# andrewmilson/ecfft

Hardware: AMD Instinct MI355X
Metric: secp256k1 Fp field-mul/s, ENTER+EXIT at n=2^20 (higher is better)
Workload: dtype u256; 1 GPU; secp256k1::Fp n=2^20 ENTER+EXIT (BASELINE.json configs[2]); n=1048576, field=secp256k1, parallelism=1 independent polynomial(s), one per GPU, no collective, inputs=device-resident (HBM) before the timed region, steps=449, warmup=5

## Files before the change

### ecfft_amd/csrc/device_tree.h

```cpp
#pragma once
#include <hip/hip_runtime.h>
#include <vector>
#include <set>
#include <map>
#include <mutex>
#include <atomic>
#include <cstdio>
#include <cstdlib>
#include <new>
#include <algorithm>
#include "kernels.h"
#include "host_curve.h"
#include "transport.h"

namespace ecfft {

#ifdef ECFFT_TEST_HOOKS
inline const char* ab_env(const char* name) { return getenv(name); }
#else
inline const char* ab_env(const char*) { return nullptr; }
#endif

#define ECFFT_HIP_TRY(x)                                                                   \
    do { hipError_t e_ = (x); if (e_ != hipSuccess) {                                      \
// ... 68 lines not shown
public:
    using E = typename F::elem;
    using TE = typename F::telem;
    using Tree = LevelTables<F>;

    ~DeviceChain() { release(); }

    size_t size() const { return N_; }
    unsigned log_size() const { return L_; }
    const Tree& tree(unsigned log_m) const { return trees_[log_m]; }
    const Tree& tree_at(unsigned log_m) const { return (ovr_tree_ && ovr_tree_->log_m == log_m) ? *ovr_tree_ : trees_[log_m]; }
    const HostTree<F>& host() const { return host_; }
    int exit_cores() const { return exit3_ ? 3 : 4; }
    int exit_low_cores() const { return exit3_ && kExitLowForm == 3 && !exit_low4_ ? 3 : 4; }
    int sym_bfly() const { return !sym_ ? 0 : (sym_general_kernels_ ? 2 : 1); }
    int low_map(int dir) const {
        if (trees_.size() > 5 && trees_[5].low32_A[dir]) return 32;
        if (trees_.size() > 4 && trees_[4].low16_A[dir]) return 16;
        return 0;
    }
    const E* f_device() const { return f_; }
    std::mutex& lock() { return mu_; }
#ifdef ECFFT_TEST_HOOKS
    static std::atomic<int>& test_fail_build_rank() { static std::atomic<int> r{-1}; return r; }
#endif
    Profiler& profiler() const { return prof_; }

    bool build(HostTree<F>&& ht, int device) {
        host_ = std::move(ht);
        N_ = host_.n; L_ = ilog2(N_); device_ = device;
// ... 522 lines not shown
    static constexpr unsigned kLogTileMax = (sizeof(E) == 32) ? ECFFT_LOG_TILE_BYTES - 5 : ECFFT_LOG_TILE_BYTES - 2;
#ifndef ECFFT_COL_STAGES
#define ECFFT_COL_STAGES 9
#endif
#ifndef ECFFT_LOG_COL_TILE_BYTES
#define ECFFT_LOG_COL_TILE_BYTES 15
#endif
#ifndef ECFFT_COL_MIN_LOGC
#define ECFFT_COL_MIN_LOGC 1
#endif
#ifndef ECFFT_COL_STAGES_4B
#define ECFFT_COL_STAGES_4B 9
#endif
    static constexpr unsigned kColStages = sizeof(E) == 4 ? ECFFT_COL_STAGES_4B : ECFFT_COL_STAGES;
    static constexpr bool kSymKernels = sizeof(E) == 32 && ECFFT_SYM_BFLY != 0;
    static constexpr unsigned kLogColTileMax = (sizeof(E) == 32) ? ECFFT_LOG_COL_TILE_BYTES - 5 : ECFFT_LOG_COL_TILE_BYTES - 2;
    struct NextLoad { int ld_mode; const TE* ld_tbl; double extra_first; };
    struct EnterFuse { const E* src; E* dst; double extra; };
    bool extend_core(unsigned log_m, IoDesc<F> io, E* buf, size_t total, int srcpar, hipStream_t s,
                     double extra_first = 0.0, double extra_last = 0.0, unsigned k_begin = 0,
                     const NextLoad* next_ld = nullptr, bool skip_first_col = false, const EnterFuse* ef = nullptr) const {
        const Tree& T = tree_at(log_m);
        size_t e = T.e; unsigned le = ilog2(e);
        int tgt = 1 - srcpar;
        const bool symk = kSymKernels && sym_kernels();
        unsigned tz = (unsigned)__builtin_ctzll((unsigned long long)total);
        unsigned log_tile = tz < kLogTileMax ? tz : kLogTileMax;
        const bool small = small_launch(total) && !ef_small_off_;
        if (small && log_tile > kLogLowSmall) log_tile = kLogLowSmall;
        unsigned k_first = le > log_tile ? le - log_tile : 0;
// ... 547 lines not shown
        enter_rec(in, X, n / 2, s, sA, depth - 1, next_side);
        double w = tblw_; tblw_ = 0.0; enter_rec(in + n / 2, X + n / 2, n / 2, s2, sB, depth - 1, next_side); tblw_ = w;
        (void)hipEventRecord(ev_join_[me], s2); (void)hipStreamWaitEvent(s, ev_join_[me], 0);
        enter_levels(X, out, n, 1, s, sA, ln, ln);
    }
    static size_t scratch_need(size_t n, unsigned depth) { return depth == 0 ? 3 * n : n + 2 * scratch_need(n / 2, depth - 1) > 4 * n ? n + 2 * scratch_need(n / 2, depth - 1) : 4 * n; }
    void enter_levels(const E* in, E* out, size_t n, size_t count, hipStream_t s, E* base, unsigned l_begin, unsigned l_end) const {
        const size_t nt = n * count;
        E* bufA = base; E* bufB = base + nt; E* work = base + 2 * nt;
        const E* src = in;
        unsigned l0 = l_begin;
        const unsigned ll = log_low_for(nt);
        if (l_begin == 1 && l_end >= ll) {
            E* dst = (l_end == ll && out != in) ? out : bufA;
            double bytes = 0; for (unsigned l = 1; l <= ll; ++l) bytes += enter_level_alg_bytes(nt, l);
            if (ll == kLogLow)
                ECFFT_LAUNCH(KC_FUSED_ENTER, bytes, (k_enter_low<F, (int)kLogLow>), dim3((unsigned)(nt >> kLogLow)), dim3(kBlockLds),
                             2 * (sizeof(E) << kLogLow), s, dst, src, (const Tree*)d_trees_);
            else
                ECFFT_LAUNCH(KC_FUSED_ENTER, bytes, (k_enter_low<F, (int)kLogLowSmall, 2 * (int)kBlockLowSmall>), dim3((unsigned)(nt >> kLogLowSmall)), dim3(2 * kBlockLowSmall),
                             2 * (sizeof(E) << kLogLowSmall), s, dst, src, (const Tree*)d_trees_);
            src = dst; l0 = ll + 1;
        }
        for (unsigned l = l0; l <= l_end; ++l) {
            const Tree& T = trees_[l];
            size_t e = T.e;
            E* dst = (l == l_end && out != in) ? out : (src == bufA ? bufB : bufA);
            IoDesc<F> io = io_plain(src, work); io.ld_mode = LD_SCALE; io.ld_tbl = T.winv[0];
            EnterFuse ef{src, dst, sizeof(E) * (3.0 * nt + 2.0 * e * tblw_)};
            extend_core(l, io, work, nt, 0, s, 0.0, 0.0, 0, nullptr, false, &ef);
            src = dst;
// ... 6 lines not shown
    }
    double exit_level_alg_bytes(size_t n, unsigned l) const {
        double e = (double)((size_t)1 << (l - 1));
        return sizeof(E) * (8.0 * (l - 1) * (double)n + 8.5 * (double)n + tblw_ * (32.0 * (e - 1) + 8.5 * e));
    }
#ifndef ECFFT_SPLIT_MIN_LOG
#define ECFFT_SPLIT_MIN_LOG 19
#endif
#ifndef ECFFT_EXIT_CORES
#define ECFFT_EXIT_CORES 3
#endif
#ifndef ECFFT_EXIT_LOW_CORES
#define ECFFT_EXIT_LOW_CORES 3
#endif
    static constexpr int kExitLowForm = (ECFFT_EXIT_CORES == 4 || ECFFT_EXIT_LOW_CORES == 4) ? 4 : 3;
    static constexpr unsigned kSplitMinLog = ECFFT_SPLIT_MIN_LOG;
#ifndef ECFFT_SPLIT_DEPTH
#define ECFFT_SPLIT_DEPTH 1
#endif
#ifndef ECFFT_NT_STORE_MAX_LOG
#define ECFFT_NT_STORE_MAX_LOG 0
#endif
    static constexpr unsigned kNtStoreMaxLog = ECFFT_NT_STORE_MAX_LOG;
    static constexpr unsigned kSplitDepth = ECFFT_SPLIT_DEPTH;
    static constexpr int kMaxSides = 7;
    static constexpr unsigned kLogLow = (sizeof(E) == 32) ? 10 : 13;
    static constexpr unsigned kLogLowSmall = 8, kBlockLowSmall = 128, kSmallTiles = 256;
    unsigned small_tiles_max() const {
        static const int v = ab_env("ECFFT_SMALL_TILES_MAX") ? atoi(ab_env("ECFFT_SMALL_TILES_MAX")) : -1;
        return v >= 0 ? (unsigned)v : (in_halves_ ? kSmallTiles : 2 * kSmallTiles);
// ... 67 lines not shown
            bool f2 = extend_core(l, io_plain(G, G), G, nh, 1, s, 0.0, 0.0, 0, &nl3, f1);
            IoDesc<F> io3 = io_plain(G, G);
            io3.ld_mode = LD_SCALE; io3.ld_tbl = T.C1;
            io3.st_mode = ST_AXPBY; io3.st_a = T.NB2; io3.st_b = T.D1; io3.aux = H; io3.aux_stride = 1; io3.aux_off = 0; io3.aux_out = nullptr;
            bool f3 = extend_core(l, io3, G, nh, 0, s, f2 ? 0.0 : se * (3.0 * n + 3.0 * ee), se * (1.5 * n + 2.0 * ee), 0, &nl4, f2);
            IoDesc<F> io4 = io_plain(G, dst);
            io4.st_mode = ST_EXIT_SPLIT; io4.st_a = T.w[0]; io4.st_b = T.xie; io4.aux = cur; io4.aux_stride = 2; io4.aux_off = 0;
            extend_core(l, io4, G, nh, 1, s, 0.0, se * (1.5 * n + 0.5 * ee), 0, nullptr, f3);
            cur = dst;
        }
        if (l_to == 1 && l_from >= ll) {
            E* dst = out != in ? out : (cur == bufA ? bufB : bufA);
            double bytes = 0; for (unsigned l = 1; l <= ll; ++l) bytes += exit_level_alg_bytes(n, l);
            const bool low3 = exit_low_cores() == 3;
            if (ll == kLogLow) {
                if (low3) ECFFT_LAUNCH(KC_FUSED_EXIT, bytes, (k_exit_low<F, (int)kLogLow, (int)kBlockLds, kExitLowForm>), dim3((unsigned)(n >> kLogLow)), dim3(kBlockLds),
                                       2 * (sizeof(E) << kLogLow), s, dst, cur, (const Tree*)d_trees_);
                else ECFFT_LAUNCH(KC_FUSED_EXIT, bytes, (k_exit_low<F, (int)kLogLow, (int)kBlockLds, 4>), dim3((unsigned)(n >> kLogLow)), dim3(kBlockLds),
                                  2 * (sizeof(E) << kLogLow), s, dst, cur, (const Tree*)d_trees_);
            } else {
                if (low3) ECFFT_LAUNCH(KC_FUSED_EXIT, bytes, (k_exit_low<F, (int)kLogLowSmall, (int)kBlockLowSmall, kExitLowForm>), dim3((unsigned)(n >> kLogLowSmall)), dim3(kBlockLowSmall),
                                       2 * (sizeof(E) << kLogLowSmall), s, dst, cur, (const Tree*)d_trees_);
                else ECFFT_LAUNCH(KC_FUSED_EXIT, bytes, (k_exit_low<F, (int)kLogLowSmall, (int)kBlockLowSmall, 4>), dim3((unsigned)(n >> kLogLowSmall)), dim3(kBlockLowSmall),
                                  2 * (sizeof(E) << kLogLowSmall), s, dst, cur, (const Tree*)d_trees_);
            }
            cur = dst;
        }
        if (cur != out) (void)hipMemcpyAsync(out, cur, n * sizeof(E), hipMemcpyDeviceToDevice, s);
    }

    bool poly_mul(const E* a, size_t na, const E* b, size_t nb, E* out, size_t count, hipStream_t s) {
// ... 2523 lines not shown
                         ~StripeScope() { ch->stripe_stage_ = nullptr; ch->stripe_bytes_ = 0; } };
    bool stripe_off_ = ab_env("ECFFT_NO_STRIPE") != nullptr;
    size_t stripe_gain_ = ab_env("ECFFT_STRIPE_MIN_GAIN") ? (size_t)atoll(ab_env("ECFFT_STRIPE_MIN_GAIN")) : ~(size_t)0;
    bool q2_split_ = ab_env("ECFFT_SPLIT_Q2_SPLIT") != nullptr;
    bool col256_off_ = ab_env("ECFFT_NO_COL256") != nullptr;
    bool row256_off_ = ab_env("ECFFT_NO_ROW256") != nullptr;
    bool ef_small_off_ = ab_env("ECFFT_NO_SMALL_TILES") != nullptr;
    bool exit4_ = ECFFT_EXIT_CORES == 4 || ab_env("ECFFT_EXIT_FOUR_CORES") != nullptr;
    bool exit3_ = false;
    bool exit_low4_ = ab_env("ECFFT_EXIT_LOW_FOUR_CORES") != nullptr;
    E* crit_ = nullptr;
    bool sym_ = false;
    bool sym_off_ = ab_env("ECFFT_NO_SYM_BFLY") != nullptr;
    bool sym_general_kernels_ = ab_env("ECFFT_SYM_BFLY_GENERAL_KERNELS") != nullptr;
    bool sym_kernels() const { return sym_ && !sym_general_kernels_; }
};

}
```

### ecfft_amd/csrc/ecfft_capi.hip

```cpp
#include <hip/hip_runtime.h>
#include <cstring>
#include <memory>
#include <new>
#include "device_tree.h"
#include "wire_parse.h"
#include "../../include/ecfft_hip.h"
#ifdef ECFFT_TEST_HOOKS
#include "../../include/ecfft_hip_hooks.h"
#endif

using namespace ecfft;

struct ecfft_ctx {
    int field;
    int device;
    std::unique_ptr<DeviceChain<Secp256k1>> secp;
    std::unique_ptr<DeviceChain<M31>> m31;
    void* stage = nullptr;
    size_t stage_bytes = 0;
    hipEvent_t last_op = nullptr;
    ~ecfft_ctx() { if (stage) (void)hipFree(stage); if (last_op) (void)hipEventDestroy(last_op); }
};

namespace {
// ... 1510 lines not shown
int ecfft_ctx_low_map(const ecfft_ctx* ctx, int dir) {
    if (!ctx || dir < 0 || dir > 1 || ctx->field != ECFFT_FIELD_SECP256K1 || !ctx->secp) return 0;
    return ctx->secp->low_map(dir);
}
int ecfft_ctx_exit_cores(const ecfft_ctx* ctx) {
    if (!ctx) return 0;
    return ctx->secp ? ctx->secp->exit_cores() : ctx->m31 ? ctx->m31->exit_cores() : 0;
}
int ecfft_ctx_exit_low_cores(const ecfft_ctx* ctx) {
    if (!ctx) return 0;
    return ctx->secp ? ctx->secp->exit_low_cores() : ctx->m31 ? ctx->m31->exit_low_cores() : 0;
}
int ecfft_ctx_sym_bfly(const ecfft_ctx* ctx) {
    if (!ctx) return -1;
    return ctx->secp ? ctx->secp->sym_bfly() : ctx->m31 ? ctx->m31->sym_bfly() : -1;
}

#endif
int ecfft_mul_ceiling(int field, int device, int waves_per_simd, double* mul_per_s) {
    return with_field(field, [&](auto tag) { return run_mul_ceiling<typename decltype(tag)::type>(device, waves_per_simd, mul_per_s); });
}

int ecfft_device_alloc(int device, size_t bytes, void** out) {
    if (!out) return ECFFT_ERR_BAD_ARG;
    *out = nullptr;
    if (!have_device(device)) return ECFFT_ERR_HIP;
    DeviceGuard dev(device);
    if (!dev.ok) return ECFFT_ERR_HIP;
    return hipMalloc(out, bytes ? bytes : 1) == hipSuccess ? ECFFT_OK : ECFFT_ERR_HIP;
}
// ... 447 lines not shown
```

### ecfft_amd/csrc/kernels.h

```cpp
#pragma once
#include <hip/hip_runtime.h>
#include <stdint.h>
#include <stddef.h>
#include <type_traits>
#include "mfma_blk16.h"
#include "curve_points.h"

namespace ecfft {

constexpr int kBlock = 256;

__device__ __forceinline__ void lds_barrier() { asm volatile("s_waitcnt lgkmcnt(0)\n\ts_barrier" ::: "memory"); }
#ifndef ECFFT_WAVE_LOCAL
#define ECFFT_WAVE_LOCAL 1
#endif
__device__ __forceinline__ void wave_local_sync() {
#if ECFFT_WAVE_LOCAL == 2
    asm volatile("s_waitcnt lgkmcnt(0)" ::: "memory");
#elif ECFFT_WAVE_LOCAL == 1
    __builtin_amdgcn_fence(__ATOMIC_ACQ_REL, "wavefront");
    asm volatile("" ::: "memory");
#else
    lds_barrier();
#endif
// ... 504 lines not shown
}

template <class F, int EPT, int BLK>
__device__ __forceinline__ void lds_extend_fast(typename F::elem* a, const typename F::telem* __restrict__ np0, const typename F::telem* __restrict__ dinv,
                                                const typename F::telem* __restrict__ p0, const typename F::telem* __restrict__ p1,
                                                const typename F::telem* __restrict__ inner, size_t e64, uint32_t log_span, uint32_t tid) {
    const uint32_t e = (uint32_t)e64;
    constexpr uint32_t LOG_EPT = EPT == 16 ? 4 : 3;
    const uint32_t upper = log_span > LOG_EPT ? log_span - LOG_EPT : 0;
    if (upper) flat_stages<F, true, EPT, BLK>(a, np0, dinv, e, LOG_EPT, upper, tid);
    tail_stages<F, EPT, BLK>(a, np0, dinv, p0, p1, inner, e, log_span, tid);
    if (upper) flat_stages<F, false, EPT, BLK>(a, p0, p1, e, LOG_EPT, upper, tid);
    __syncthreads();
}

template <class F, bool DEC, bool SYM = false>
__device__ __forceinline__ void row_stages_pipe(typename F::elem* tile, const typename F::telem* __restrict__ ta, const typename F::telem* __restrict__ tb,
                                                uint32_t e, int lh_from, int lh_to, uint32_t tid, int lh_after = 99) {
    using E = typename F::elem;
    using TE = typename F::telem;
    if (DEC ? lh_from < lh_to : lh_from > lh_to) return;
    auto geom = [&](int lh, uint32_t& idx, uint32_t& ti) {
        const uint32_t h = 1u << lh, i = tid & (h - 1);
        idx = ((tid >> lh) << (lh + 1)) + i; ti = e - 2 * h + i;
    };
    uint32_t idx, ti;
    geom(lh_from, idx, ti);
    if constexpr (SYM) {
        const TE* __restrict__ tk = DEC ? tb : ta;
        TE nk = ldt(tk, ti);
#pragma unroll 1
        for (int lh = lh_from; DEC ? lh >= lh_to : lh <= lh_to; lh += DEC ? -1 : 1) {
            const TE t = nk;
            const uint32_t lo = idx, up = idx + (1u << lh);
            E a = tile[lo], b = tile[up];
            sym_bfly<F, DEC>(a, b, t);
            tile[lo] = a; tile[up] = b;
            if (lh != lh_to) { geom(lh + (DEC ? -1 : 1), idx, ti); nk = ldt(tk, ti); }
            const int nxt = lh != lh_to ? lh + (DEC ? -1 : 1) : lh_after;
            if (wave_local_lh(lh) && wave_local_lh(nxt)) wave_local_sync(); else lds_barrier();
        }
        return;
    }
    TE na = ldt(ta, ti), nb = ldt(tb, ti);
#pragma unroll 1
    for (int lh = lh_from; DEC ? lh >= lh_to : lh <= lh_to; lh += DEC ? -1 : 1) {
        const TE t0 = na, t1 = nb;
        const uint32_t lo = idx, up = idx + (1u << lh);
        const E a = tile[lo], b = tile[up];
        if (DEC) { const E q1 = F::tmul(t1, F::sub(b, a)); tile[lo] = F::tmul_add(t0, q1, a); tile[up] = q1; }
        else { const E o0 = F::tmul_add(t0, b, a), o1 = F::tmul_add(t1, b, a); tile[lo] = o0; tile[up] = o1; }
        if (lh != lh_to) { geom(lh + (DEC ? -1 : 1), idx, ti); na = ldt(ta, ti); nb = ldt(tb, ti); }
        const int nxt = lh != lh_to ? lh + (DEC ? -1 : 1) : lh_after;
// ... 827 lines not shown
        const uint32_t lh = log_e - k - 1, h = 1u << lh;
        const bool hi = (tid >> lh) & 1u;
        const uint32_t off = (uint32_t)(e - 2 * (size_t)h) + (tid & (h - 1));
        TE t; if (act) t = hi ? ldt(p1, off) : ldt(p0, off);
        const E xp = partner(h);
        if (act) {
            const E A = lane_sel<F>(hi, xp, x), B = lane_sel<F>(hi, x, xp);
            x = F::tmul_add(t, B, A);
        }
    }
    __syncthreads();
    if (act) lds_put<F, SWZ>(a, tid, x);
    __syncthreads();
}

template <class F, int BLK = kBlockLds, bool SWZ = false>
__device__ __forceinline__ void lds_extend_core(typename F::elem* a, uint32_t len, uint32_t log_e, const LevelTables<F>& T, int srcpar) {
    using E = typename F::elem;
    uint32_t tid_ = threadIdx.x;
#if ECFFT_CORE_OPAQUE_TID
    if constexpr (sizeof(E) == 32) asm volatile("" : "+v"(tid_));
#endif
    const uint32_t tid = tid_, npairs = len >> 1;
    const size_t e = (size_t)1 << log_e;
    const int tgt = 1 - srcpar;
    const uint8_t* bA = nullptr; const unsigned long long* bK = nullptr;
    if constexpr (sizeof(E) == 32 && BLK == 512) {
        if (log_e >= 4 && (len == 512u || (len & 1023u) == 0)) { bA = T.blk16_A[srcpar]; bK = T.blk16_K[srcpar]; }
    }
    if constexpr (sizeof(E) == 32 && (BLK == 256 || BLK == 128)) {
        if (log_e >= 4 && len == (uint32_t)BLK) { bA = T.blk16_A[srcpar]; bK = T.blk16_K[srcpar]; }
    }
    if constexpr (sizeof(E) == 32 && ECFFT_REG_ENGINE) {
        if (len <= (uint32_t)BLK && (len & 63u) == 0) {
            reg_extend32<F, BLK, SWZ>(a, len, log_e, 0, T.c0t[srcpar], T.dinv[srcpar], T.p0[tgt], T.p1[tgt], T.inner[srcpar], tid, len == (uint32_t)BLK ? bA : nullptr, bK);
            return;
        }
    }
    if constexpr (SWZ) __builtin_trap();
    if constexpr (sizeof(E) == 32) {
        if (len == BLK) {
            const uint32_t g = tid & (npairs - 1);
            const bool hi = tid >= npairs;
            const uint32_t k_inner = log_e ? log_e - 1 : 0;
            for (uint32_t k = 0; k < k_inner; ++k) {
                const uint32_t lh = log_e - k - 1, h = 1u << lh, i = g & (h - 1), idx = ((g >> lh) << (lh + 1)) + i;
// ... 21 lines not shown
                a[idx + (hi ? h : 0)] = F::tmul_add(t, y, x);
                __syncthreads();
            }
            return;
        }
    }
    if constexpr (sizeof(E) == 4) {
        if (len == BLK * 16) { lds_extend_fast<F, 16, BLK>(a, T.np0[srcpar], T.dinv[srcpar], T.p0[tgt], T.p1[tgt], T.inner[srcpar], e, log_e, tid); return; }
        if (len == BLK * 8) { lds_extend_fast<F, 8, BLK>(a, T.np0[srcpar], T.dinv[srcpar], T.p0[tgt], T.p1[tgt], T.inner[srcpar], e, log_e, tid); return; }
    }
    const uint32_t k_inner = log_e ? log_e - 1 : 0;
    bool mfma = false;
    if constexpr (sizeof(E) == 32 && BLK == 512) mfma = bA != nullptr && (len & 1023u) == 0;
    const uint32_t k_dec_end = mfma ? log_e - 4 : k_inner;
    const bool wl = sizeof(E) == 32 && 2 * npairs > (uint32_t)BLK;
    for (uint32_t k = 0; k < k_dec_end; ++k) {
        const uint32_t lh = log_e - k - 1, h = 1u << lh;
        stage_sweep<F, true, BLK>(a, T.np0[srcpar] + (e - 2 * (size_t)h), T.dinv[srcpar] + (e - 2 * (size_t)h), lh, npairs, tid, T.c0t[srcpar] + (e - 2 * (size_t)h));
        if (wl && wave_local_lh((int)lh) && (k + 1 < k_dec_end || !mfma)) wave_local_sync(); else __syncthreads();
    }
    if constexpr (sizeof(E) == 32 && BLK == 512) {
        if (mfma) {
            Blk16::APre pre = Blk16::prefetch(bA, tid);
            __builtin_amdgcn_sched_barrier(0);
            Blk16::to_operand_form<BLK>(a, len, tid);
#pragma unroll 1
            for (uint32_t o = 0; o < len; o += Blk16::kSub) {
                if (o) { pre = Blk16::prefetch(bA, tid); __builtin_amdgcn_sched_barrier(0); }
                Blk16::phase(a + o, bA, bK, tid, pre);
            }
            Blk16::from_swizzled<BLK>(a, len, tid);
        }
    }
    if (log_e > 0 && !mfma) {
        const typename F::telem c0 = ldt(T.inner[srcpar], 0u), c1 = ldt(T.inner[srcpar], 1u);
        for (uint32_t g = tid; g < npairs; g += BLK) {
            E x = a[2 * g], y = a[2 * g + 1];
            E d = F::sub(y, x);
            a[2 * g] = F::tmul_add(c0, d, x);
            a[2 * g + 1] = F::tmul_add(c1, d, x);
        }
        if (wl && ECFFT_WAVE_LOCAL && k_dec_end > 0) wave_local_sync(); else __syncthreads();
    }
    for (uint32_t k = k_dec_end; k-- > 0;) {
        const uint32_t lh = log_e - k - 1, h = 1u << lh;
        stage_sweep<F, false, BLK>(a, T.p0[tgt] + (e - 2 * (size_t)h), T.p1[tgt] + (e - 2 * (size_t)h), lh, npairs, tid);
        if (wl && k > 0 && wave_local_lh((int)lh + 1)) wave_local_sync(); else __syncthreads();
    }
}

template <class F, int LOG_TILE, int BLK = kBlockLds>
__global__ __launch_bounds__(BLK, (BLK >= 512 ? ECFFT_MIN_WAVES : 2)) void k_enter_low(typename F::elem* __restrict__ dst, const typename F::elem* __restrict__ src,
                                                          const LevelTables<F>* __restrict__ trees) {
    using E = typename F::elem;
    extern __shared__ __attribute__((aligned(16))) unsigned char ecfft_smem[];
    constexpr uint32_t log_tile = LOG_TILE, T = 1u << LOG_TILE, npairs = T >> 1;
    constexpr bool kRoles = npairs * 2 == (uint32_t)BLK;
    constexpr int PAIRS = kRoles ? 1 : (int)(npairs / BLK);
    static_assert(kRoles || (npairs >= (uint32_t)BLK && npairs % BLK == 0), "tile too small for the workgroup");
    const uint32_t tid = threadIdx.x;
    E* cur = reinterpret_cast<E*>(ecfft_smem);
    E* work = cur + T;
    const size_t base = (size_t)blockIdx.x << log_tile;
    constexpr bool kQuad = sizeof(E) == 4 && T % (4 * BLK) == 0;
    bool qio = false;
    if constexpr (kQuad) qio = ((reinterpret_cast<uintptr_t>(src) | reinterpret_cast<uintptr_t>(dst)) & 15) == 0;
// ... 76 lines not shown
                            if (k < 2) { lo[c].v[2 * k] = ev; lo[c].v[2 * k + 1] = od; } else { hi[c].v[2 * (k - 2)] = ev; hi[c].v[2 * (k - 2) + 1] = od; }
                        }
                }
                __syncthreads();
#pragma unroll
                for (int c = 0; c < NP; ++c) {
                    const uint32_t g = 4u * (tid + (uint32_t)c * BLK), i = g & (e - 1), bb = (g >> le) << l;
                    stq(cur + bb + 2 * i, lo[c]); stq(cur + bb + 2 * i + 4, hi[c]);
                }
                __syncthreads();
                continue;
            }
        }
        for (uint32_t j = tid; j < T; j += BLK) work[j] = F::tmul(ldt(L.winv[0], j & (e - 1)), cur[j]);
        __syncthreads();
        lds_extend_core<F, BLK>(work, T, le, L, 0);
        if constexpr (kRoles) {
            const bool hi = tid >= npairs;
            const uint32_t g = hi ? tid - npairs : tid, i = g & (e - 1), bb = (g >> le) << l;
            E r;
            if (!hi) r = F::tmul_add(ldt(L.xe, i), cur[bb + e + i], cur[bb + i]);
            else r = F::tmul_add(ldt(L.w1x, i), work[bb + e + i], F::tmul(ldt(L.w[1], i), work[bb + i]));
            __syncthreads();
            cur[bb + 2 * i + (hi ? 1 : 0)] = r;
            __syncthreads();
            continue;
        }
        E ev[PAIRS], od[PAIRS];
#pragma unroll
        for (int c = 0; c < PAIRS; ++c) {
            uint32_t g = tid + (uint32_t)c * BLK, i = g & (e - 1), bb = (g >> le) << l;
// ... 13 lines not shown
        if (qio) {
            constexpr int NQ = (int)(T / (4 * BLK));
#pragma unroll
            for (int c = 0; c < NQ; ++c) {
                Quad q = ldq(cur + 4u * (tid + (uint32_t)c * BLK));
#pragma unroll
                for (int k = 0; k < 4; ++k) q.v[k] = F::canon(q.v[k]);
                stq(dst + base + 4u * (tid + (uint32_t)c * BLK), q);
            }
            return;
        }
    }
    for (uint32_t j = tid; j < T; j += BLK) dst[base + j] = F::canon(cur[j]);
}

template <class F, int LOG_TILE, int BLK = kBlockLds, int CORES = 4>
__global__ __launch_bounds__(BLK, (BLK >= 512 ? ECFFT_MIN_WAVES : 1)) void k_exit_low(typename F::elem* __restrict__ dst, const typename F::elem* __restrict__ src,
                                                         const LevelTables<F>* __restrict__ trees) {
    using E = typename F::elem;
    static_assert(CORES == 3 || CORES == 4, "three or four EXTEND cores per level");
    constexpr bool k3 = CORES == 3;
    constexpr int par1 = k3 ? 1 : 0;
    extern __shared__ __attribute__((aligned(16))) unsigned char ecfft_smem[];
    constexpr uint32_t log_tile = LOG_TILE, T = 1u << LOG_TILE, nh = T >> 1;
    constexpr int PAIRS = (int)(nh / BLK);
    static_assert(PAIRS >= 1 && nh % BLK == 0, "tile too small for the workgroup");
    const uint32_t tid = threadIdx.x;
    E* cur = reinterpret_cast<E*>(ecfft_smem);
    E* G = cur + T;
    E* H = G + nh;
    const size_t base = (size_t)blockIdx.x << log_tile;
// ... 104 lines not shown
#pragma unroll
                        for (int k = 0; k < 4; ++k) { uq[c].v[k] = F::tmul(ta[c].v[k], x[c].v[k]); vq[c].v[k] = F::tmul(tb[c].v[k], F::sub(y[c].v[k], uq[c].v[k])); }
                }
                __syncthreads();
#pragma unroll
                for (int c = 0; c < NP; ++c) {
                    const uint32_t g = gq(c), i = g & (e - 1), bb = (g >> le) << l;
                    stq(cur + bb + i, uq[c]); stq(cur + bb + e + i, vq[c]);
                }
                __syncthreads();
                continue;
            }
        }
        for (uint32_t g = tid; g < nh; g += BLK) lds_put<F, kSwz>(G, g, F::tmul(ldt(k3 ? L.zA1 : L.A1, g & (e - 1)), lds_get<F, kSwz>(cur, 2 * g + par1)));
        __syncthreads();
        lds_extend_core<F, BLK, kSwz>(G, nh, le, L, par1);
        for (uint32_t g = tid; g < nh; g += BLK) {
            uint32_t i = g & (e - 1);
            E r = F::tmul_add(ldt(k3 ? L.zNB2 : L.NB2, i), lds_get<F, kSwz>(G, g), F::tmul(ldt(k3 ? L.zB1 : L.B1, i), lds_get<F, kSwz>(cur, 2 * g + 1 - par1)));
            lds_put<F, kSwz>(G, g, r); lds_put<F, kSwz>(H, g, r);
        }
        __syncthreads();
        lds_extend_core<F, BLK, kSwz>(G, nh, le, L, 1 - par1);
        for (uint32_t g = tid; g < nh; g += BLK) lds_put<F, kSwz>(G, g, F::tmul(ldt(k3 ? L.zC1 : L.C1, g & (e - 1)), lds_get<F, kSwz>(G, g)));
        __syncthreads();
        lds_extend_core<F, BLK, kSwz>(G, nh, le, L, par1);
        if constexpr (!k3) {
            for (uint32_t g = tid; g < nh; g += BLK) {
                uint32_t i = g & (e - 1);
                lds_put<F, kSwz>(G, g, F::tmul_add(ldt(L.NB2, i), lds_get<F, kSwz>(G, g), F::tmul(ldt(L.D1, i), lds_get<F, kSwz>(H, g))));
            }
            __syncthreads();
            lds_extend_core<F, BLK, kSwz>(G, nh, le, L, 1);
        }
        E u[PAIRS], v[PAIRS];
#pragma unroll
        for (int c = 0; c < PAIRS; ++c) {
            uint32_t g = tid + (uint32_t)c * BLK, i = g & (e - 1);
            if constexpr (k3) u[c] = F::tmul_add(ldt(L.zNB3, i), lds_get<F, kSwz>(G, g), F::tmul(ldt(L.zD1, i), lds_get<F, kSwz>(H, g)));
            else u[c] = F::tmul(ldt(L.w[0], i), lds_get<F, kSwz>(G, g));
            v[c] = F::tmul(ldt(L.xie, i), F::sub(lds_get<F, kSwz>(cur, 2 * g), u[c]));
        }
        __syncthreads();
#pragma unroll
        for (int c = 0; c < PAIRS; ++c) {
            uint32_t g = tid + (uint32_t)c * BLK, i = g & (e - 1), bb = (g >> le) << l;
            lds_put<F, kSwz>(cur, bb + i, u[c]); lds_put<F, kSwz>(cur, bb + e + i, v[c]);
        }
// ... 1660 lines not shown
```

### ecfft_amd/fftree.py

```python
import ctypes
import enum
import os

import numpy as np

from . import build as _build

_DIR = os.path.dirname(os.path.abspath(__file__))

OK, ERR_NOT_POW2, ERR_TREE_TOO_SMALL, ERR_TREE_TOO_LARGE, ERR_HIP, ERR_BAD_ARG = range(6)
MEM_HOST, MEM_DEVICE = 0, 1
TBL_F, TBL_RECOMBINE, TBL_DECOMPOSE, TBL_XNN_S, TBL_XNN_S_INV, TBL_Z0_S1, TBL_Z1_S0, TBL_Z0_INV_S1, TBL_Z1_INV_S0, TBL_Z0Z0, TBL_Z1Z1 = range(11)

EXPORTS = ["ecfft_elem_size", "ecfft_build_fftree", "ecfft_fftree_new", "ecfft_ctx_destroy", "ecfft_tree_size",
           "ecfft_field", "ecfft_enter", "ecfft_exit", "ecfft_extend", "ecfft_tree_table", "ecfft_build_points",
           "ecfft_device_info", "ecfft_profile_enable", "ecfft_profile_classes", "ecfft_profile_read",
           "ecfft_extend_top_cyclic", "ecfft_extend_local_block",
           "ecfft_mul_ceiling", "ecfft_elems_to_standard", "ecfft_elems_from_standard", "ecfft_table_fma", "ecfft_enter_many", "ecfft_exit_many", "ecfft_mextend", "ecfft_redc", "ecfft_modular_reduce", "ecfft_vanish", "ecfft_degree",
           "ecfft_comm_get_unique_id", "ecfft_comm_init_rank", "ecfft_comm_init_callback", "ecfft_comm_destroy", "ecfft_comm_rank", "ecfft_comm_world",
           "ecfft_comm_stats_enable", "ecfft_comm_stats_read", "ecfft_extend_sharded", "ecfft_enter_sharded", "ecfft_exit_sharded", "ecfft_device_copy", "ecfft_shader_clock", "ecfft_device_alloc", "ecfft_device_free", "ecfft_device_sync", "ecfft_build_extend_shard", "ecfft_ctx_device_bytes", "ecfft_extend_sharded_layout", "ecfft_build_enter_shard", "ecfft_build_exit_shard", "ecfft_build_exit_shard_opts",
           "ecfft_fftree_serialize", "ecfft_fftree_deserialize", "ecfft_tree_rational_maps", "ecfft_ctx_trim", "ecfft_comm_abort", "ecfft_comm_set_rccl_library", "ecfft_comm_set_link_striping",
           "ecfft_poly_mul", "ecfft_poly_inv_series", "ecfft_poly_divrem", "ecfft_poly_eval_points", "ecfft_poly_interpolate",
           "ecfft_poly_pow_mod", "ecfft_poly_mul_mod", "ecfft_poly_gcd", "ecfft_poly_xgcd", "ecfft_poly_xgcd_partial", "ecfft_rs_decode", "ecfft_poly_find_roots",
           "ecfft_poly_compose_mod", "ecfft_poly_squarefree", "ecfft_poly_distinct_degree", "ecfft_poly_equal_degree", "ecfft_division_polynomial", "ecfft_curve_trace_mod", "ecfft_curve_cardinality",
           "ecfft_find_curve_candidate", "ecfft_curve_two_sylow", "ecfft_find_curve", "ecfft_build_fftree_on_curve",
           "ecfft_curve_point_mul", "ecfft_curve_point_two_adicity", "ecfft_curve_find_generator", "ecfft_build_ec_fftree"]
GCD_SMALL_MAX = 256
XGCD_PARTIAL_SMALL_MAX = 256
RS_SMALL_MAX = 255
ROOTS_SMALL_MAX = 65
COMPOSE_SMALL_MAX = 65
DDF_SMALL_MAX = 65
EDF_SMALL_MAX = 65
SCHOOF_SMALL_MAX = 65
SCHOOF_MAX_L = 199
ORDER_BYTES = 40

HOOK_EXPORTS = ['ecfft_selftest_field', 'ecfft_selfcheck_pointwise_z', 'ecfft_test_fail_next_collective', 'ecfft_selftest_blk16', 'ecfft_selftest_blk16_small', 'ecfft_test_fail_build_rank', 'ecfft_comm_init_projection', 'ecfft_selftest_blk32', 'ecfft_ctx_low_map', 'ecfft_curve_search_stats', 'ecfft_test_ddf_iterate', 'ecfft_test_schoof_pi2', 'ecfft_ctx_exit_cores', 'ecfft_ctx_exit_low_cores', 'ecfft_ctx_sym_bfly']

EXCHANGE_FN = ctypes.CFUNCTYPE(ctypes.c_int, ctypes.c_void_p, ctypes.c_int, ctypes.POINTER(ctypes.c_int), ctypes.POINTER(ctypes.c_void_p),
                               ctypes.POINTER(ctypes.c_size_t), ctypes.c_int, ctypes.POINTER(ctypes.c_int), ctypes.POINTER(ctypes.c_void_p),
                               ctypes.POINTER(ctypes.c_size_t), ctypes.c_void_p)


class Moiety(enum.IntEnum):
    S0 = 0
    S1 = 1


class EcfftError(RuntimeError):
    pass


# ... 89 lines not shown
    L.ecfft_comm_set_link_striping.restype, L.ecfft_comm_set_link_striping.argtypes = ci, [vp, sz]
    L.has_hooks = hasattr(L, "ecfft_selftest_field")
    if L.has_hooks:
        L.ecfft_selftest_field.restype, L.ecfft_selftest_field.argtypes = ci, [ci, ci, vp, vp, vp, vp, sz, ci]
        L.ecfft_selfcheck_pointwise_z.restype, L.ecfft_selfcheck_pointwise_z.argtypes = ctypes.c_long, [vp, sz]
        L.ecfft_test_fail_next_collective.restype, L.ecfft_test_fail_next_collective.argtypes = ci, [vp]
        L.ecfft_test_fail_build_rank.restype, L.ecfft_test_fail_build_rank.argtypes = ci, [ci]
        L.ecfft_selftest_blk16.restype, L.ecfft_selftest_blk16.argtypes = ci, [vp, vp, vp, sz, ci]
        L.ecfft_selftest_blk16_small.restype, L.ecfft_selftest_blk16_small.argtypes = ci, [vp, vp, vp, sz, ci, ci]
        L.ecfft_selftest_blk32.restype, L.ecfft_selftest_blk32.argtypes = ci, [vp, vp, vp, sz, ci]
        L.ecfft_ctx_low_map.restype, L.ecfft_ctx_low_map.argtypes = ci, [vp, ci]
        L.ecfft_ctx_exit_cores.restype, L.ecfft_ctx_exit_cores.argtypes = ci, [vp]
        L.ecfft_ctx_exit_low_cores.restype, L.ecfft_ctx_exit_low_cores.argtypes = ci, [vp]
        if hasattr(L, "ecfft_ctx_sym_bfly"):
            L.ecfft_ctx_sym_bfly.restype, L.ecfft_ctx_sym_bfly.argtypes = ci, [vp]
        L.ecfft_curve_search_stats.restype, L.ecfft_curve_search_stats.argtypes = ci, [ctypes.POINTER(ctypes.c_uint64), ctypes.POINTER(ctypes.c_double), sz, ci]
        L.ecfft_test_ddf_iterate.restype, L.ecfft_test_ddf_iterate.argtypes = ci, [ci]
        L.ecfft_test_schoof_pi2.restype, L.ecfft_test_schoof_pi2.argtypes = ci, [ci]
        L.ecfft_comm_init_projection.restype = ci
        L.ecfft_comm_init_projection.argtypes = [ci, ci, ci, ctypes.c_double, ctypes.c_double, ctypes.POINTER(vp)]
    return L


def _load(path):
    try:
        import torch
    except ImportError:
        pass
    return _bind(ctypes.CDLL(path))

# ... 723 lines not shown
    def exit_sharded(self, comm, y_block, n):
        return self._sharded(self._L.ecfft_exit_sharded, comm, y_block, n)

    def low_map(self, direction):
        return self._L.ecfft_ctx_low_map(self._h, int(direction))

    def exit_cores(self):
        return self._L.ecfft_ctx_exit_cores(self._h)

    def exit_low_cores(self):
        return self._L.ecfft_ctx_exit_low_cores(self._h)

    def sym_bfly(self):
        return self._L.ecfft_ctx_sym_bfly(self._h)

    def profile(self, on):
        _check(self._L.ecfft_profile_enable(self._h, int(on)))

    def profile_read(self):
        out = []
        for c in range(self._L.ecfft_profile_classes()):
            name = ctypes.create_string_buffer(64); n = ctypes.c_uint64(); ms = ctypes.c_double(); by = ctypes.c_double()
            _check(self._L.ecfft_profile_read(self._h, c, name, 64, ctypes.byref(n), ctypes.byref(ms), ctypes.byref(by)))
            out.append({"name": name.value.decode(), "launches": n.value, "ms": ms.value, "alg_bytes": by.value})
        return out

    def table(self, which, m=None):
        m = self.n if m is None else m
        cnt = ctypes.c_size_t()
        _check(self._L.ecfft_tree_table(self._h, m, which, None, 0, ctypes.byref(cnt)))
# ... 57 lines not shown
```

### include/ecfft_hip_hooks.h

```cpp
#ifndef ECFFT_HIP_HOOKS_H
#define ECFFT_HIP_HOOKS_H
#include "ecfft_hip.h"
#ifdef __cplusplus
extern "C" {
#endif

long ecfft_selfcheck_pointwise_z(ecfft_ctx* ctx, size_t m);

int ecfft_comm_init_projection(int world, int rank, int device, double delay_us, double link_gbps, ecfft_comm** out);

int ecfft_test_fail_next_collective(ecfft_ctx* ctx);
int ecfft_test_fail_build_rank(int rank);

int ecfft_selftest_field(int field, int op, const void* a, const void* b, const void* c, void* out, size_t n, int device);

int ecfft_selftest_blk16(const void* matrix256, const void* x, void* out, size_t n, int device);
int ecfft_selftest_blk16_small(const void* matrix256, const void* x, void* out, size_t n, int mode, int device);
int ecfft_selftest_blk32(const void* matrix1024, const void* x, void* out, size_t n, int device);
int ecfft_ctx_low_map(const ecfft_ctx* ctx, int dir);
int ecfft_ctx_exit_cores(const ecfft_ctx* ctx);
int ecfft_ctx_exit_low_cores(const ecfft_ctx* ctx);
int ecfft_ctx_sym_bfly(const ecfft_ctx* ctx);
int ecfft_curve_search_stats(uint64_t* lens, double* seconds, size_t cap, int reset);

int ecfft_test_ddf_iterate(int mode);

int ecfft_test_schoof_pi2(int mode);

#ifdef __cplusplus
}
#endif
#endif
```

Before: 567.9 billion field-mul/s.

## Use symmetric butterflies in fused low-level enter and exit LDS kernels

Adds SYM template variants of k_enter_low and k_exit_low. For 512-thread tiles these replace the generic stage_sweep decompose and recompose loops in lds_extend_core with pipelined symmetric-butterfly stages (row_stages_pipe, plus a new half-thread pair_extend512 path for the exit). Both are enabled by default for 32-byte elements when the symmetric kernels are active. The aim is to cut field multiplications and table loads per butterfly in the fused low levels. In exchange the exit path leaves half the threads idle during butterfly stages and adds more template instantiations and register pressure.

After: 584.0 billion field-mul/s, median of 6. +2.8%, better.

```diff
diff --git a/ecfft_amd/csrc/device_tree.h b/ecfft_amd/csrc/device_tree.h
--- a/ecfft_amd/csrc/device_tree.h
+++ b/ecfft_amd/csrc/device_tree.h
@@ -106,6 +106,7 @@
     int exit_cores() const { return exit3_ ? 3 : 4; }
     int exit_low_cores() const { return exit3_ && kExitLowForm == 3 && !exit_low4_ ? 3 : 4; }
     int sym_bfly() const { return !sym_ ? 0 : (sym_general_kernels_ ? 2 : 1); }
+    int low_sym() const { return (kLowSymEnter && low_sym_enter() ? 1 : 0) | (kLowSymExit && low_sym_exit() ? 2 : 0); }
     int low_map(int dir) const {
         if (trees_.size() > 5 && trees_[5].low32_A[dir]) return 32;
         if (trees_.size() > 4 && trees_[4].low16_A[dir]) return 16;
@@ -658,6 +659,7 @@
 #endif
     static constexpr unsigned kColStages = sizeof(E) == 4 ? ECFFT_COL_STAGES_4B : ECFFT_COL_STAGES;
     static constexpr bool kSymKernels = sizeof(E) == 32 && ECFFT_SYM_BFLY != 0;
+    static constexpr bool kLowSymEnter = kSymKernels && ECFFT_ENTER_LOW_SYM != 0;
     static constexpr unsigned kLogColTileMax = (sizeof(E) == 32) ? ECFFT_LOG_COL_TILE_BYTES - 5 : ECFFT_LOG_COL_TILE_BYTES - 2;
     struct NextLoad { int ld_mode; const TE* ld_tbl; double extra_first; };
     struct EnterFuse { const E* src; E* dst; double extra; };
@@ -1235,7 +1237,10 @@
         if (l_begin == 1 && l_end >= ll) {
             E* dst = (l_end == ll && out != in) ? out : bufA;
             double bytes = 0; for (unsigned l = 1; l <= ll; ++l) bytes += enter_level_alg_bytes(nt, l);
-            if (ll == kLogLow)
+            if (ll == kLogLow && kLowSymEnter && low_sym_enter())
+                ECFFT_LAUNCH(KC_FUSED_ENTER, bytes, (k_enter_low<F, (int)kLogLow, (int)kBlockLds, kLowSymEnter>), dim3((unsigned)(nt >> kLogLow)), dim3(kBlockLds),
+                             2 * (sizeof(E) << kLogLow), s, dst, src, (const Tree*)d_trees_);
+            else if (ll == kLogLow)
                 ECFFT_LAUNCH(KC_FUSED_ENTER, bytes, (k_enter_low<F, (int)kLogLow>), dim3((unsigned)(nt >> kLogLow)), dim3(kBlockLds),
                              2 * (sizeof(E) << kLogLow), s, dst, src, (const Tree*)d_trees_);
             else
@@ -1272,6 +1277,7 @@
 #define ECFFT_EXIT_LOW_CORES 3
 #endif
     static constexpr int kExitLowForm = (ECFFT_EXIT_CORES == 4 || ECFFT_EXIT_LOW_CORES == 4) ? 4 : 3;
+    static constexpr bool kLowSymExit = kSymKernels && ECFFT_EXIT_LOW_SYM != 0 && kExitLowForm == 3;
     static constexpr unsigned kSplitMinLog = ECFFT_SPLIT_MIN_LOG;
 #ifndef ECFFT_SPLIT_DEPTH
 #define ECFFT_SPLIT_DEPTH 1
@@ -1369,7 +1375,10 @@
             double bytes = 0; for (unsigned l = 1; l <= ll; ++l) bytes += exit_level_alg_bytes(n, l);
             const bool low3 = exit_low_cores() == 3;
             if (ll == kLogLow) {
-                if (low3) ECFFT_LAUNCH(KC_FUSED_EXIT, bytes, (k_exit_low<F, (int)kLogLow, (int)kBlockLds, kExitLowForm>), dim3((unsigned)(n >> kLogLow)), dim3(kBlockLds),
+                if (low3 && kLowSymExit && low_sym_exit())
+                    ECFFT_LAUNCH(KC_FUSED_EXIT, bytes, (k_exit_low<F, (int)kLogLow, (int)kBlockLds, kExitLowForm, kLowSymExit>), dim3((unsigned)(n >> kLogLow)), dim3(kBlockLds),
+                                 2 * (sizeof(E) << kLogLow), s, dst, cur, (const Tree*)d_trees_);
+                else if (low3) ECFFT_LAUNCH(KC_FUSED_EXIT, bytes, (k_exit_low<F, (int)kLogLow, (int)kBlockLds, kExitLowForm>), dim3((unsigned)(n >> kLogLow)), dim3(kBlockLds),
                                        2 * (sizeof(E) << kLogLow), s, dst, cur, (const Tree*)d_trees_);
                 else ECFFT_LAUNCH(KC_FUSED_EXIT, bytes, (k_exit_low<F, (int)kLogLow, (int)kBlockLds, 4>), dim3((unsigned)(n >> kLogLow)), dim3(kBlockLds),
                                   2 * (sizeof(E) << kLogLow), s, dst, cur, (const Tree*)d_trees_);
@@ -3923,6 +3932,9 @@
     bool sym_off_ = ab_env("ECFFT_NO_SYM_BFLY") != nullptr;
     bool sym_general_kernels_ = ab_env("ECFFT_SYM_BFLY_GENERAL_KERNELS") != nullptr;
     bool sym_kernels() const { return sym_ && !sym_general_kernels_; }
+    bool low_general_kernels_ = ab_env("ECFFT_LOW_GENERAL_KERNELS") != nullptr;
+    bool low_sym_enter() const { return sym_kernels() && !low_general_kernels_ && !exit4_; }
+    bool low_sym_exit() const { return low_sym_enter() && exit_low_cores() == 3; }
 };
 
 }
diff --git a/ecfft_amd/csrc/ecfft_capi.hip b/ecfft_amd/csrc/ecfft_capi.hip
--- a/ecfft_amd/csrc/ecfft_capi.hip
+++ b/ecfft_amd/csrc/ecfft_capi.hip
@@ -1548,6 +1548,10 @@
 int ecfft_ctx_sym_bfly(const ecfft_ctx* ctx) {
     if (!ctx) return -1;
     return ctx->secp ? ctx->secp->sym_bfly() : ctx->m31 ? ctx->m31->sym_bfly() : -1;
+}
+int ecfft_ctx_low_sym(const ecfft_ctx* ctx) {
+    if (!ctx) return -1;
+    return ctx->secp ? ctx->secp->low_sym() : ctx->m31 ? ctx->m31->low_sym() : -1;
 }
 
 #endif
diff --git a/ecfft_amd/csrc/kernels.h b/ecfft_amd/csrc/kernels.h
--- a/ecfft_amd/csrc/kernels.h
+++ b/ecfft_amd/csrc/kernels.h
@@ -542,7 +542,7 @@
     __syncthreads();
 }
 
-template <class F, bool DEC, bool SYM = false>
+template <class F, bool DEC, bool SYM = false, bool PIPE = true>
 __device__ __forceinline__ void row_stages_pipe(typename F::elem* tile, const typename F::telem* __restrict__ ta, const typename F::telem* __restrict__ tb,
                                                 uint32_t e, int lh_from, int lh_to, uint32_t tid, int lh_after = 99) {
     using E = typename F::elem;
@@ -556,15 +556,17 @@
     geom(lh_from, idx, ti);
     if constexpr (SYM) {
         const TE* __restrict__ tk = DEC ? tb : ta;
-        TE nk = ldt(tk, ti);
+        TE nk;
+        if constexpr (PIPE) nk = ldt(tk, ti);
 #pragma unroll 1
         for (int lh = lh_from; DEC ? lh >= lh_to : lh <= lh_to; lh += DEC ? -1 : 1) {
+            if constexpr (!PIPE) nk = ldt(tk, ti);
             const TE t = nk;
             const uint32_t lo = idx, up = idx + (1u << lh);
             E a = tile[lo], b = tile[up];
             sym_bfly<F, DEC>(a, b, t);
             tile[lo] = a; tile[up] = b;
-            if (lh != lh_to) { geom(lh + (DEC ? -1 : 1), idx, ti); nk = ldt(tk, ti); }
+            if (lh != lh_to) { geom(lh + (DEC ? -1 : 1), idx, ti); if constexpr (PIPE) nk = ldt(tk, ti); }
             const int nxt = lh != lh_to ? lh + (DEC ? -1 : 1) : lh_after;
             if (wave_local_lh(lh) && wave_local_lh(nxt)) wave_local_sync(); else lds_barrier();
         }
@@ -1422,7 +1424,58 @@
     __syncthreads();
 }
 
-template <class F, int BLK = kBlockLds, bool SWZ = false>
+#ifndef ECFFT_EXIT_LOW_SYM
+#define ECFFT_EXIT_LOW_SYM 1
+#endif
+#ifndef ECFFT_EXIT_LOW_SYM_WAVES
+#define ECFFT_EXIT_LOW_SYM_WAVES 0
+#endif
+template <class F, bool DEC, bool SWZ>
+__device__ __forceinline__ void half_stages_pipe(typename F::elem* a, const typename F::telem* __restrict__ tk, uint32_t e, int lh_from, int lh_to,
+                                                 uint32_t q, bool sw) {
+    using E = typename F::elem;
+    using TE = typename F::telem;
+    auto geom = [&](int lh, uint32_t& idx, uint32_t& ti) {
+        const uint32_t h = 1u << lh, i = q & (h - 1);
+        idx = ((q >> lh) << (lh + 1)) + i; ti = e - 2 * h + i;
+    };
+    uint32_t idx = 0, ti = 0;
+    TE nk;
+    if (sw) { geom(lh_from, idx, ti); nk = ldt(tk, ti); }
+#pragma unroll 1
+    for (int lh = lh_from; DEC ? lh >= lh_to : lh <= lh_to; lh += DEC ? -1 : 1) {
+        if (sw) {
+            const TE t = nk;
+            const uint32_t lo = idx, up = idx + (1u << lh);
+            E x = lds_get<F, SWZ>(a, lo), y = lds_get<F, SWZ>(a, up);
+            sym_bfly<F, DEC>(x, y, t);
+            lds_put<F, SWZ>(a, lo, x); lds_put<F, SWZ>(a, up, y);
+            if (lh != lh_to) { geom(lh + (DEC ? -1 : 1), idx, ti); nk = ldt(tk, ti); }
+        }
+        const int nxt = lh != lh_to ? lh + (DEC ? -1 : 1) : 99;
+        if (wave_local_lh(lh) && wave_local_lh(nxt)) wave_local_sync(); else lds_barrier();
+    }
+}
+template <class F, bool SWZ>
+__device__ __forceinline__ void pair_extend512(typename F::elem* a, uint32_t log_e, const typename F::telem* __restrict__ dinv, const typename F::telem* __restrict__ p0,
+                                               uint32_t tid, const uint8_t* __restrict__ blkA, const unsigned long long* __restrict__ blkK) {
+    using E = typename F::elem;
+    const bool sw = ECFFT_EXIT_LOW_SYM_WAVES ? ((tid >> 6) & 1u) == 0 : tid < 256u;
+    const uint32_t q = ECFFT_EXIT_LOW_SYM_WAVES ? (((tid >> 7) << 6) | (tid & 63u)) : (tid & 255u);
+    const uint32_t e = 1u << log_e;
+    half_stages_pipe<F, true, SWZ>(a, dinv, e, (int)log_e - 1, 4, q, sw);
+    E x = lds_get<F, SWZ>(a, tid);
+    x = Blk16::phase512_regs(a, x, blkA, blkK, tid);
+    __syncthreads();
+    lds_put<F, SWZ>(a, tid, x);
+    __syncthreads();
+    half_stages_pipe<F, false, SWZ>(a, p0, e, 4, (int)log_e - 1, q, sw);
+}
+
+#ifndef ECFFT_ENTER_LOW_SYM
+#define ECFFT_ENTER_LOW_SYM 1
+#endif
+template <class F, int BLK = kBlockLds, bool SWZ = false, bool SYM = false>
 __device__ __forceinline__ void lds_extend_core(typename F::elem* a, uint32_t len, uint32_t log_e, const LevelTables<F>& T, int srcpar) {
     using E = typename F::elem;
     uint32_t tid_ = threadIdx.x;
@@ -1438,6 +1491,9 @@
     }
     if constexpr (sizeof(E) == 32 && (BLK == 256 || BLK == 128)) {
         if (log_e >= 4 && len == (uint32_t)BLK) { bA = T.blk16_A[srcpar]; bK = T.blk16_K[srcpar]; }
+    }
+    if constexpr (SYM && sizeof(E) == 32 && BLK == 512 && ECFFT_EXIT_LOW_SYM != 0) {
+        if (len == (uint32_t)BLK && bA && log_e >= 5) { pair_extend512<F, SWZ>(a, log_e, T.dinv[srcpar], T.p0[tgt], tid, bA, bK); return; }
     }
     if constexpr (sizeof(E) == 32 && ECFFT_REG_ENGINE) {
         if (len <= (uint32_t)BLK && (len & 63u) == 0) {
@@ -1489,6 +1545,12 @@
     if constexpr (sizeof(E) == 32 && BLK == 512) mfma = bA != nullptr && (len & 1023u) == 0;
     const uint32_t k_dec_end = mfma ? log_e - 4 : k_inner;
     const bool wl = sizeof(E) == 32 && 2 * npairs > (uint32_t)BLK;
+    bool symp = false;
+    if constexpr (SYM && sizeof(E) == 32 && BLK == 512) {
+        symp = mfma && npairs == (uint32_t)BLK;
+        if (symp) row_stages_pipe<F, true, true, ECFFT_ENTER_LOW_SYM != 2>(a, T.np0[srcpar], T.dinv[srcpar], (uint32_t)e, (int)log_e - 1, 4, tid);
+    }
+    if (!symp)
     for (uint32_t k = 0; k < k_dec_end; ++k) {
         const uint32_t lh = log_e - k - 1, h = 1u << lh;
         stage_sweep<F, true, BLK>(a, T.np0[srcpar] + (e - 2 * (size_t)h), T.dinv[srcpar] + (e - 2 * (size_t)h), lh, npairs, tid, T.c0t[srcpar] + (e - 2 * (size_t)h));
@@ -1517,6 +1579,9 @@
         }
         if (wl && ECFFT_WAVE_LOCAL && k_dec_end > 0) wave_local_sync(); else __syncthreads();
     }
+    if constexpr (SYM && sizeof(E) == 32 && BLK == 512) {
+        if (symp) { row_stages_pipe<F, false, true, ECFFT_ENTER_LOW_SYM != 2>(a, T.p0[tgt], T.p1[tgt], (uint32_t)e, 4, (int)log_e - 1, tid); return; }
+    }
     for (uint32_t k = k_dec_end; k-- > 0;) {
         const uint32_t lh = log_e - k - 1, h = 1u << lh;
         stage_sweep<F, false, BLK>(a, T.p0[tgt] + (e - 2 * (size_t)h), T.p1[tgt] + (e - 2 * (size_t)h), lh, npairs, tid);
@@ -1524,7 +1589,7 @@
     }
 }
 
-template <class F, int LOG_TILE, int BLK = kBlockLds>
+template <class F, int LOG_TILE, int BLK = kBlockLds, bool SYM = false>
 __global__ __launch_bounds__(BLK, (BLK >= 512 ? ECFFT_MIN_WAVES : 2)) void k_enter_low(typename F::elem* __restrict__ dst, const typename F::elem* __restrict__ src,
                                                           const LevelTables<F>* __restrict__ trees) {
     using E = typename F::elem;
@@ -1631,7 +1696,7 @@
         }
         for (uint32_t j = tid; j < T; j += BLK) work[j] = F::tmul(ldt(L.winv[0], j & (e - 1)), cur[j]);
         __syncthreads();
-        lds_extend_core<F, BLK>(work, T, le, L, 0);
+        lds_extend_core<F, BLK, false, SYM>(work, T, le, L, 0);
         if constexpr (kRoles) {
             const bool hi = tid >= npairs;
             const uint32_t g = hi ? tid - npairs : tid, i = g & (e - 1), bb = (g >> le) << l;
@@ -1675,7 +1740,7 @@
     for (uint32_t j = tid; j < T; j += BLK) dst[base + j] = F::canon(cur[j]);
 }
 
-template <class F, int LOG_TILE, int BLK = kBlockLds, int CORES = 4>
+template <class F, int LOG_TILE, int BLK = kBlockLds, int CORES = 4, bool SYM = false>
 __global__ __launch_bounds__(BLK, (BLK >= 512 ? ECFFT_MIN_WAVES : 1)) void k_exit_low(typename F::elem* __restrict__ dst, const typename F::elem* __restrict__ src,
                                                          const LevelTables<F>* __restrict__ trees) {
     using E = typename F::elem;
@@ -1810,24 +1875,24 @@
         }
         for (uint32_t g = tid; g < nh; g += BLK) lds_put<F, kSwz>(G, g, F::tmul(ldt(k3 ? L.zA1 : L.A1, g & (e - 1)), lds_get<F, kSwz>(cur, 2 * g + par1)));
         __syncthreads();
-        lds_extend_core<F, BLK, kSwz>(G, nh, le, L, par1);
+        lds_extend_core<F, BLK, kSwz, SYM && k3>(G, nh, le, L, par1);
         for (uint32_t g = tid; g < nh; g += BLK) {
             uint32_t i = g & (e - 1);
             E r = F::tmul_add(ldt(k3 ? L.zNB2 : L.NB2, i), lds_get<F, kSwz>(G, g), F::tmul(ldt(k3 ? L.zB1 : L.B1, i), lds_get<F, kSwz>(cur, 2 * g + 1 - par1)));
             lds_put<F, kSwz>(G, g, r); lds_put<F, kSwz>(H, g, r);
         }
         __syncthreads();
-        lds_extend_core<F, BLK, kSwz>(G, nh, le, L, 1 - par1);
+        lds_extend_core<F, BLK, kSwz, SYM && k3>(G, nh, le, L, 1 - par1);
         for (uint32_t g = tid; g < nh; g += BLK) lds_put<F, kSwz>(G, g, F::tmul(ldt(k3 ? L.zC1 : L.C1, g & (e - 1)), lds_get<F, kSwz>(G, g)));
         __syncthreads();
-        lds_extend_core<F, BLK, kSwz>(G, nh, le, L, par1);
+        lds_extend_core<F, BLK, kSwz, SYM && k3>(G, nh, le, L, par1);
         if constexpr (!k3) {
             for (uint32_t g = tid; g < nh; g += BLK) {
                 uint32_t i = g & (e - 1);
                 lds_put<F, kSwz>(G, g, F::tmul_add(ldt(L.NB2, i), lds_get<F, kSwz>(G, g), F::tmul(ldt(L.D1, i), lds_get<F, kSwz>(H, g))));
             }
             __syncthreads();
-            lds_extend_core<F, BLK, kSwz>(G, nh, le, L, 1);
+            lds_extend_core<F, BLK, kSwz, SYM && k3>(G, nh, le, L, 1);
         }
         E u[PAIRS], v[PAIRS];
 #pragma unroll
diff --git a/ecfft_amd/fftree.py b/ecfft_amd/fftree.py
--- a/ecfft_amd/fftree.py
+++ b/ecfft_amd/fftree.py
@@ -36,7 +36,7 @@
 SCHOOF_MAX_L = 199
 ORDER_BYTES = 40
 
-HOOK_EXPORTS = ['ecfft_selftest_field', 'ecfft_selfcheck_pointwise_z', 'ecfft_test_fail_next_collective', 'ecfft_selftest_blk16', 'ecfft_selftest_blk16_small', 'ecfft_test_fail_build_rank', 'ecfft_comm_init_projection', 'ecfft_selftest_blk32', 'ecfft_ctx_low_map', 'ecfft_curve_search_stats', 'ecfft_test_ddf_iterate', 'ecfft_test_schoof_pi2', 'ecfft_ctx_exit_cores', 'ecfft_ctx_exit_low_cores', 'ecfft_ctx_sym_bfly']
+HOOK_EXPORTS = ['ecfft_selftest_field', 'ecfft_selfcheck_pointwise_z', 'ecfft_test_fail_next_collective', 'ecfft_selftest_blk16', 'ecfft_selftest_blk16_small', 'ecfft_test_fail_build_rank', 'ecfft_comm_init_projection', 'ecfft_selftest_blk32', 'ecfft_ctx_low_map', 'ecfft_curve_search_stats', 'ecfft_test_ddf_iterate', 'ecfft_test_schoof_pi2', 'ecfft_ctx_exit_cores', 'ecfft_ctx_exit_low_cores', 'ecfft_ctx_sym_bfly', 'ecfft_ctx_low_sym']
 
 EXCHANGE_FN = ctypes.CFUNCTYPE(ctypes.c_int, ctypes.c_void_p, ctypes.c_int, ctypes.POINTER(ctypes.c_int), ctypes.POINTER(ctypes.c_void_p),
                                ctypes.POINTER(ctypes.c_size_t), ctypes.c_int, ctypes.POINTER(ctypes.c_int), ctypes.POINTER(ctypes.c_void_p),
@@ -156,6 +156,8 @@
         L.ecfft_ctx_exit_low_cores.restype, L.ecfft_ctx_exit_low_cores.argtypes = ci, [vp]
         if hasattr(L, "ecfft_ctx_sym_bfly"):
             L.ecfft_ctx_sym_bfly.restype, L.ecfft_ctx_sym_bfly.argtypes = ci, [vp]
+        if hasattr(L, "ecfft_ctx_low_sym"):
+            L.ecfft_ctx_low_sym.restype, L.ecfft_ctx_low_sym.argtypes = ci, [vp]
         L.ecfft_curve_search_stats.restype, L.ecfft_curve_search_stats.argtypes = ci, [ctypes.POINTER(ctypes.c_uint64), ctypes.POINTER(ctypes.c_double), sz, ci]
         L.ecfft_test_ddf_iterate.restype, L.ecfft_test_ddf_iterate.argtypes = ci, [ci]
         L.ecfft_test_schoof_pi2.restype, L.ecfft_test_schoof_pi2.argtypes = ci, [ci]
@@ -909,6 +911,9 @@
     def sym_bfly(self):
         return self._L.ecfft_ctx_sym_bfly(self._h)
 
+    def low_sym(self):
+        return self._L.ecfft_ctx_low_sym(self._h)
+
     def profile(self, on):
         _check(self._L.ecfft_profile_enable(self._h, int(on)))
 
diff --git a/include/ecfft_hip_hooks.h b/include/ecfft_hip_hooks.h
--- a/include/ecfft_hip_hooks.h
+++ b/include/ecfft_hip_hooks.h
@@ -21,6 +21,7 @@
 int ecfft_ctx_exit_cores(const ecfft_ctx* ctx);
 int ecfft_ctx_exit_low_cores(const ecfft_ctx* ctx);
 int ecfft_ctx_sym_bfly(const ecfft_ctx* ctx);
+int ecfft_ctx_low_sym(const ecfft_ctx* ctx);
 int ecfft_curve_search_stats(uint64_t* lens, double* seconds, size_t cap, int reset);
 
 int ecfft_test_ddf_iterate(int mode);
```
